# dataexplorations2026/cough_detector

Measured on AMD Instinct MI355X. Metric: 1s@16kHz clips/sec (featurise+infer), higher is better.
Workload: dtype bf16x3: split-bf16 MFMA (feature image, activations and BN-folded weights as hi+lo bf16 pairs, 3 v_mfma_f32_32x32x16_bf16 per k-step, f32 accumulate, f32 activations in HBM); featuriser f32

## Files before the change

### cough_detector_amd/csrc/featurize.hip

```cpp
#include <cmath>
#include <cstddef>
#include <cstring>
#include <type_traits>
#include <vector>

#include <hip/hip_bf16.h>

#include <cstdlib>

#include "common.h"
#include "fft256.h"
#include "internal.h"

namespace cough {
namespace {

constexpr int NS = 16000, NFFT = 512, HOP = 160, WIN = 400, NFRAMES = 101, NMEL = 64, NMFCC = 13;
constexpr int PADL = NFFT / 2;
constexpr int NBIN = 128;
constexpr int MAXW = 8;
constexpr int THREADS = 256, WAVES = THREADS / 64;
constexpr int FPW = 4;
constexpr int NGROUP = (NFRAMES + FPW - 1) / FPW;
constexpr int XROW = 17;
constexpr int XFRAME = 16 * XROW;
constexpr int NMF = NMFCC * NFRAMES;
constexpr int FIRST_PLAIN = 2, LAST_PLAIN = 98;

struct FeatTables {
    float win[NFFT];
    float2 tw256[16][16];
    float2 tw512[NBIN];
    int mel_start[NMEL];
    float mel_w[NMEL][MAXW];
    float dct_t[NMFCC + 1][NMEL];
};

constexpr size_t LDS_XCH = size_t(WAVES) * FPW * XFRAME * 4;
constexpr size_t LDS_MEL = size_t(NMEL) * NFRAMES * 4;
constexpr size_t LDS_RED = 16 * 4;
constexpr size_t LDS_TW = size_t(16) * XROW * 8;
constexpr size_t LDS_TOTAL = LDS_XCH + LDS_MEL + LDS_RED + LDS_TW;
static_assert(LDS_TOTAL * 3 <= 160 * 1024, "three workgroups per CU");
static_assert(LDS_XCH >= size_t(2) * NMF * 4, "MFCC / delta buffers alias the transpose scratch");

__device__ __forceinline__ float block_max(float v, float* red, int tid) {
    v = wave_max(v);
    __syncthreads();
    if ((tid & 63) == 0) red[tid >> 6] = v;
    __syncthreads();
    float r = red[0];
#pragma unroll
    for (int w = 1; w < WAVES; ++w) r = fmaxf(r, red[w]);
    return r;
}
__device__ __forceinline__ float block_sum(float v, float* red, int tid) {
    v = wave_sum(v);
    __syncthreads();
    if ((tid & 63) == 0) red[tid >> 6] = v;
    __syncthreads();
    float r = red[0];
#pragma unroll
    for (int w = 1; w < WAVES; ++w) r += red[w];
    return r;
}

#ifdef COUGH_K1_STAMPS
__device__ unsigned long long* g_stamp_buf = nullptr;
#define K1_STAMP(slot)                                                                      \
    do {                                                                                    \
        if (g_stamp_buf && threadIdx.x == 0)                                                \
            g_stamp_buf[(size_t)blockIdx.x * 8 + (slot)] = __builtin_amdgcn_s_memtime();    \
    } while (0)
#else
#define K1_STAMP(slot) do { } while (0)
#endif

#ifdef COUGH_K1_MARKERS
#define K1_MARK(text)                             \
    do {                                          \
        __builtin_amdgcn_sched_barrier(0);        \
        asm volatile("; K1MARK " text);           \
        __builtin_amdgcn_sched_barrier(0);        \
    } while (0)
#else
#define K1_MARK(text) do { } while (0)
#endif

using f32x16 = __attribute__((ext_vector_type(16))) float;
using bf16x8 = __attribute__((ext_vector_type(8))) __bf16;
__device__ __forceinline__ uint16_t f2bf(float f) {
    __hip_bfloat16 b = __float2bfloat16(f);
    return *reinterpret_cast<uint16_t*>(&b);
}
constexpr int ST_P1H = 22, ST_P1W = 25, ST_ROWS = 94, ST_PITCH = 106;
constexpr int ST_PER = ST_P1H * ST_P1W, ST_TILES = (ST_PER + 7) / 8;
constexpr size_t ST_IMG = size_t(ST_ROWS) * ST_PITCH * 2;
static_assert(ST_IMG <= LDS_MEL, "the bf16 feature image aliases the dB buffer");
constexpr size_t ST_X3_OFF = LDS_TOTAL - 2 * ST_IMG;
static_assert(ST_X3_OFF % 16 == 0 && ST_IMG % 4 == 0 && ST_X3_OFF >= size_t(NMF) * 4, "hi / lo images vs the MFCC buffer");

struct FullBank {
    int n_mels, n_mfcc, n_taps;
    int maxw[2];
    int n_frames, n_samples, hop;
    int cph, cph_pad, cw;
    const int *lo, *hi, *off;
    const float* w;
    const float* dct;
};
constexpr size_t full_mel_bytes(int n_mels, int n_frames = NFRAMES) { return (size_t(n_mels) * n_frames * 4 + 15) & ~size_t(15); }
constexpr int FX_ROW = FPW * 16 + 1, FX_WAVE = 16 * FX_ROW, FX_PROW = 260;
static_assert(FPW * FX_PROW <= FX_WAVE && FX_PROW >= NFFT / 2 + 2 && FX_PROW % 2 == 0, "four power rows replace the transposes");
constexpr size_t LDS_XCH_FULL = size_t(WAVES) * FX_WAVE * 4;
constexpr int FULL_MAX_MFCC = int(LDS_XCH_FULL / (size_t(2) * NFRAMES * 4));
constexpr size_t full_lds_bytes(int n_mels, int n_taps, int n_frames = NFRAMES) {
    return LDS_XCH_FULL + full_mel_bytes(n_mels, n_frames) + LDS_RED + LDS_TW + ((size_t(n_taps) * 4 + 15) & ~size_t(15));
}

#ifndef COUGH_GEO_WG_PER_CU
#define COUGH_GEO_WG_PER_CU 2
#endif
template <bool PRE_EMPH, int STEM, bool FULL = false, bool TALL = false, bool PCS = false, bool GEO = false>
__global__ __launch_bounds__(THREADS, GEO ? COUGH_GEO_WG_PER_CU : 3) void featurize_kernel(
    const float* __restrict__ wav, long long wav_stride, float* __restrict__ out, int nfeat,
    const FeatTables* __restrict__ tb, int normalize, float pre_coef, int delta_delta , int pcen, StemFuse stem, FullBank fbk,
    const float* __restrict__ full_dct ,
    float* __restrict__ peak_out ) {
    extern __shared__ __attribute__((aligned(16))) char smem[];
    static_assert(!GEO || (FULL && STEM == 0 && !TALL && !PCS), "run-time geometry: full-band instantiations without a stem");
    const int NF = GEO ? fbk.n_frames : NFRAMES, NGR = GEO ? (fbk.n_frames + FPW - 1) / FPW : NGROUP;
    const int NSMP = GEO ? fbk.n_samples : NS, HP = GEO ? fbk.hop : HOP;
    constexpr int N1A = GEO ? 0 : 1, N1B = GEO ? 16 : 15;
    const int nmel = FULL ? fbk.n_mels : NMEL, nmfcc = FULL ? fbk.n_mfcc : NMFCC, nmf = nmfcc * NF;
    const size_t lds_mel = FULL ? full_mel_bytes(nmel, NF) : LDS_MEL;
    constexpr size_t lds_xch = FULL ? LDS_XCH_FULL : LDS_XCH;
    float* xs = reinterpret_cast<float*>(smem);
    float* melbuf = reinterpret_cast<float*>(smem + lds_xch);
    float* red = reinterpret_cast<float*>(smem + lds_xch + lds_mel);
    float2* twl = reinterpret_cast<float2*>(smem + lds_xch + lds_mel + LDS_RED);
    float* c_w = reinterpret_cast<float*>(smem + lds_xch + lds_mel + LDS_RED + LDS_TW);

    const int tid = threadIdx.x, lane = tid & 63, wave = tid >> 6;
    const long long clip = blockIdx.x;
    const float* x = wav + clip * wav_stride;
    float* o = out + clip * (long long)nfeat * NF;
    const bool wr = out != nullptr;

    K1_STAMP(0);
    K1_STAMP(1);
    K1_MARK("PHASE prologue (window taps, twiddle table, mel taps to registers)");

    const int j = lane & 15, fsub = lane >> 4;
    twl[(tid >> 4) * XROW + (tid & 15)] = tb->tw256[tid >> 4][tid & 15];
    int b_lo[2] = {0, 0}, b_w[2] = {0, 0}, b_band[2] = {0, 0};
    const float* b_taps[2] = {c_w, c_w};
    int fpl1 = FPW;
    if constexpr (FULL) {
        for (int i = tid; i < fbk.n_taps; i += THREADS) c_w[i] = fbk.w[i];
        const int r = nmel - 64;
        fpl1 = r > 32 ? 4 : r > 16 ? 2 : 1;
#pragma unroll
        for (int ps = 0; ps < 2; ++ps) {
            const int mb = ps == 0 ? lane : 64 + (fpl1 == 4 ? lane : fpl1 == 2 ? (lane & 31) : (lane & 15));
            if (mb < nmel) {
                b_band[ps] = mb;
                b_lo[ps] = fbk.lo[mb];
                b_w[ps] = fbk.hi[mb] - b_lo[ps];
                b_taps[ps] = c_w + fbk.off[mb];
            } else {
                b_band[ps] = -1;
            }
        }
    }
    __syncthreads();
    const float2* tw_row = twl + j * XROW;
    const float2 tw_j = tb->tw512[j];
    float mw[MAXW];
#pragma unroll
    for (int q = 0; q < MAXW; ++q) mw[q] = tb->mel_w[lane][q];
    const int mstart = tb->mel_start[lane];

    float* myx = xs + (wave * FPW + fsub) * XFRAME;
    float* myw = xs + wave * FX_WAVE;
    float* fxw = myw + 16 * fsub + j;
    const float* fxr = myw + FX_ROW * j + 16 * fsub;
    float* prow = myw + FX_PROW * fsub;
    float run_max = -INFINITY;
    float peak = 0.f;
    float chk = 0.f;
    auto geo_plain = [&](int g) {
        return HP * (FPW * g) - PADL >= 0 && FPW * g + FPW - 1 < NF && HP * (FPW * g + FPW - 1) - PADL + NFFT <= NSMP;
    };
    [[maybe_unused]] float raw_left = 0.f;
    auto load_group = [&](int g, float2 (&raw)[16]) {
        const int t_raw = FPW * g + fsub;
        const int t = t_raw < NF ? t_raw : NF - 1;
        const int s0 = HP * t - PADL + 2 * j;
        if constexpr (GEO) {
            if (geo_plain(g)) {
#pragma unroll
                for (int n1 = 0; n1 < 16; ++n1) raw[n1] = make_float2(x[s0 + 32 * n1], x[s0 + 32 * n1 + 1]);
                if constexpr (PRE_EMPH) raw_left = s0 - 2 * j > 0 ? x[s0 - 2 * j - 1] : 0.f;
            } else {
#pragma unroll
                for (int n1 = 0; n1 < 16; ++n1) {
                    int i0 = s0 + 32 * n1, i1 = i0 + 1;
                    i0 = i0 < 0 ? -i0 : (i0 >= NSMP ? 2 * (NSMP - 1) - i0 : i0);
                    i1 = i1 < 0 ? -i1 : (i1 >= NSMP ? 2 * (NSMP - 1) - i1 : i1);
                    raw[n1] = make_float2(x[i0], x[i1]);
                }
            }
        } else
        if (FPW * g >= FIRST_PLAIN && FPW * g + FPW - 1 <= LAST_PLAIN) {
            K1_MARK("WEIGHT 0.885 (23 of 26 groups: frames inside the clip)");
#pragma unroll
            for (int n1 = 1; n1 < 15; ++n1) raw[n1] = *reinterpret_cast<const float2*>(x + s0 + 32 * n1);
            K1_MARK("ENDWEIGHT");
        } else {
            K1_MARK("WEIGHT 0.115 (3 of 26 groups: reflected edge frames)");
#pragma unroll
            for (int n1 = 1; n1 < 15; ++n1) {
                int i0 = s0 + 32 * n1, i1 = i0 + 1;
                i0 = i0 < 0 ? -i0 : (i0 >= NS ? 2 * (NS - 1) - i0 : i0);
                i1 = i1 < 0 ? -i1 : (i1 >= NS ? 2 * (NS - 1) - i1 : i1);
                raw[n1] = make_float2(x[i0], x[i1]);
            }
            K1_MARK("ENDWEIGHT");
        }
    };
    float2 raw[16];
    float peak_m = 0.f;
    auto p1_pass = [&](const float ws1, const float ws2) {
        float w_re[16], w_im[16];
        const int jw = 2 * j;
#pragma unroll
        for (int n1 = N1A; n1 < N1B; ++n1) {
            w_re[n1] = tb->win[32 * n1 + jw] * ws1 * ws2;
            w_im[n1] = tb->win[32 * n1 + jw + 1] * ws1 * ws2;
        }
        load_group(wave, raw);

        K1_MARK("LOOP 6.5 P1 four-frame groups per wave");
        for (int g = wave; g < NGR; g += WAVES) {
            K1_MARK("PHASE P1 peak + window multiply + next group's loads");
            const int t_raw = FPW * g + fsub;
            const int t = t_raw < NF ? t_raw : NF - 1;
            const int s0 = HP * t - PADL + 2 * j;
            float2 a[16];
            if constexpr (!GEO) {
// ... 237 lines not shown
                    float pw[26];
                    pcen_chunk(m2, c, q2, pw);
#pragma unroll
                    for (int k = 0; k < 26; ++k)
                        if (q0 + 26 * c + k < q2) o[m2 * NF + q0 + 26 * c + k] = pw[k];
                }
            }
        }
        const float mn = -block_max(-lmin, red, tid), mx = block_max(lmax, red, tid);
        const float rng = 1.0f / (mx - mn + 1e-8f);
#pragma unroll
        for (int c = 0; c < 2; ++c)
#pragma unroll
            for (int k = 0; k < 26; ++k)
                if (q0 + 26 * c + k < q1) o[m * NF + q0 + 26 * c + k] = (pv[c][k] - mn) * rng;
        for (int t = q0; t < q2; ++t) o[m2 * NF + t] = (o[m2 * NF + t] - mn) * rng;
        wr_mel = false;
    } else
    if (pcen) {
        const int m = tid >> 2, t0 = (tid & 3) * 26, t1 = t0 + 26 < NF ? t0 + 26 : NF;
        float p[36], pv[26];
#pragma unroll
        for (int k = 0; k < 36; ++k) {
            const int u = t0 - 5 + k;
            p[k] = (u >= 0 && u < NF) ? exp2f((melbuf[m * NF + u] - shift) * 0.33219280948873623f) : 0.f;
        }
        float lmin = INFINITY, lmax = -INFINITY;
        float s2[35];
#pragma unroll
        for (int k = 0; k < 35; ++k) s2[k] = p[k] + p[k + 1];
#pragma unroll
        for (int k = 0; k < 26; ++k) {
            const float sm = ((s2[k] + s2[k + 2]) + (s2[k + 4] + s2[k + 6])) + s2[k + 8];
            const float gain = __builtin_amdgcn_exp2f(-0.98f * __builtin_amdgcn_logf(1e-6f + sm * 0.1f));
            pv[k] = __builtin_amdgcn_sqrtf(fmaf(p[k + 5], gain, 2.0f)) - 1.41421356237309515f;
            if (t0 + k < t1) { lmin = fminf(lmin, pv[k]); lmax = fmaxf(lmax, pv[k]); }
        }
        const float mn = -block_max(-lmin, red, tid), mx = block_max(lmax, red, tid);
        const float rng = 1.0f / (mx - mn + 1e-8f);
        if (wr) {
#pragma unroll
            for (int k = 0; k < 26; ++k)
                if (t0 + k < t1) o[m * NF + t0 + k] = (pv[k] - mn) * rng;
        }
        if constexpr (PCS) {
#pragma unroll
            for (int k = 0; k < 26; ++k) pcv[k] = (pv[k] - mn) * rng;
        }
        wr_mel = false;
    }
    K1_MARK("ENDSKIP");
    K1_MARK("PHASE P2 floor + mel rows store");
    if constexpr (GEO) {
        for (int i = tid; i < nmel * NF; i += THREADS) {
            const float d = fmaxf(fmaxf(melbuf[i] - shift, -100.0f), floor_db);
            melbuf[i] = d;
            if (wr_mel) o[i] = fminf(fmaxf((d + 80.0f) * 0.0125f, 0.f), 1.f);
        }
    } else
    for (int i2 = tid; i2 < nmel * NFRAMES / 2; i2 += THREADS) {
        float2 d = reinterpret_cast<float2*>(melbuf)[i2];
        d.x = fmaxf(fmaxf(d.x - shift, -100.0f), floor_db);
        d.y = fmaxf(fmaxf(d.y - shift, -100.0f), floor_db);
        reinterpret_cast<float2*>(melbuf)[i2] = d;
        float2 v;
        v.x = fminf(fmaxf((d.x + 80.0f) * 0.0125f, 0.f), 1.f);
        v.y = fminf(fmaxf((d.y + 80.0f) * 0.0125f, 0.f), 1.f);
        if (wr_mel) reinterpret_cast<float2*>(o)[i2] = v;
    }
    __syncthreads();
    K1_STAMP(4);
    if (delta_delta == 2) return;
    K1_MARK("PHASE P2 DCT 13x64");
    float* mf = xs;
    float* dl = GEO ? melbuf : mf + nmf;
    const int tt0 = tid & 127;
    const int chalf = __builtin_amdgcn_readfirstlane(tid >> 7);
    if constexpr (FULL) {
        const int cph = fbk.cph, nch = chalf ? nmfcc - cph : cph, cbase = chalf * cph;
        auto dct_chunks = [&](auto cw_tag) {
            constexpr int CW = decltype(cw_tag)::value;
            for (int tt = tt0; tt < (GEO ? ((NF + 127) & ~127) : 128); tt += 128)
            for (int cq = 0; cq < nch; cq += CW) {
                float acc[CW];
#pragma unroll
                for (int cc = 0; cc < CW; ++cc) acc[cc] = 0.f;
                if (tt < NF) {
                    const float* drow = full_dct + (size_t(chalf) * fbk.cph_pad + cq) / CW * size_t(nmel) * 8;
#pragma unroll 8
                    for (int m = 0; m < nmel; ++m) {
                        const float v = melbuf[m * NF + tt];
#pragma unroll
                        for (int cc = 0; cc < CW; ++cc) acc[cc] = fmaf(drow[m * 8 + cc], v, acc[cc]);
                    }
#pragma unroll
                    for (int cc = 0; cc < CW; ++cc)
                        if (cq + cc < nch) mf[(cbase + cq + cc) * NF + tt] = acc[cc];
                }
            }
        };
        if (fbk.cw == 7) dct_chunks(std::integral_constant<int, 7>{});
        else if (fbk.cw == 6) dct_chunks(std::integral_constant<int, 6>{});
        else if (fbk.cw == 5) dct_chunks(std::integral_constant<int, 5>{});
        else dct_chunks(std::integral_constant<int, 4>{});
        __syncthreads();
        float ls = 0.f;
        for (int i = tid; i < nmf; i += THREADS) ls += mf[i];
        const float mean = block_sum(ls, red, tid) / float(nmf);
        float lq = 0.f;
        for (int i = tid; i < nmf; i += THREADS) {
            const float d = mf[i] - mean;
            lq += d * d;
        }
        const float sd = sqrtf(block_sum(lq, red, tid) / float(nmf - 1));
        const float rdenom = 1.0f / (sd + 1e-8f);
        K1_STAMP(5);
        for (int i = tid; i < nmf; i += THREADS) mf[i] = (mf[i] - mean) * rdenom;
    } else {
        const int c0 = chalf * 7, nc = chalf ? 6 : 7, tt = tt0;
        float acc[7] = {0.f, 0.f, 0.f, 0.f, 0.f, 0.f, 0.f};
        if (tt < NFRAMES) {
            const float* drow = &tb->dct_t[c0][0];
#pragma unroll 8
            for (int m = 0; m < NMEL; ++m) {
                const float v = melbuf[m * NFRAMES + tt];
#pragma unroll
                for (int cc = 0; cc < 7; ++cc) acc[cc] = fmaf(drow[cc * NMEL + m], v, acc[cc]);
            }
        }
        K1_MARK("PHASE P2 mean / std / z-score");
        float lsum = 0.f;
#pragma unroll
        for (int cc = 0; cc < 7; ++cc) lsum += (tt < NFRAMES && cc < nc) ? acc[cc] : 0.f;
        const float mean = block_sum(lsum, red, tid) / float(NMF);
        K1_STAMP(5);
        float lsq = 0.f;
#pragma unroll
        for (int cc = 0; cc < 7; ++cc) {
            const float d = acc[cc] - mean;
            lsq += (tt < NFRAMES && cc < nc) ? d * d : 0.f;
        }
        const float sd = sqrtf(block_sum(lsq, red, tid) / float(NMF - 1));
        const float rdenom = 1.0f / (sd + 1e-8f);
        if (tt < NFRAMES) {
#pragma unroll
            for (int cc = 0; cc < 7; ++cc)
                if (cc < nc) mf[(c0 + cc) * NFRAMES + tt] = (acc[cc] - mean) * rdenom;
        }
    }
    __syncthreads();
    K1_MARK("PHASE P2 feature image (stem) + MFCC / delta rows");
    uint16_t* img = STEM == 2 ? reinterpret_cast<uint16_t*>(smem + ST_X3_OFF) : reinterpret_cast<uint16_t*>(melbuf);
    uint16_t* img_lo = img + ST_ROWS * ST_PITCH;
    auto put = [&](int idx, float v) {
        const uint16_t hi = f2bf(v);
        img[idx] = hi;
        if constexpr (STEM == 2) img_lo[idx] = f2bf(v - __uint_as_float(uint32_t(hi) << 16));
    };
    if constexpr (TALL) {
        static_assert(!TALL || STEM == 2, "the 103-row stem: split-bf16 operands");
        constexpr int TL_P1H = 26, TL_HALF = 13, TL_PER = TL_HALF * ST_P1W, TL_ROWS = 58, TL_PLANE = TL_ROWS * ST_PITCH;
        constexpr size_t TL_IMG_OFF = (size_t(2) * NMF * 4 + 15) & ~size_t(15), TL_STASH_OFF = TL_IMG_OFF + size_t(2) * TL_PLANE * 2;
        constexpr int TL_KEEP0 = 2 * 2 * TL_HALF - 3;
        static_assert(TL_STASH_OFF % 16 == 0 && TL_STASH_OFF + size_t(NMEL - TL_KEEP0) * NFRAMES * 4 <= LDS_TOTAL, "103-row stem LDS");
        static_assert(2 * (2 * (TL_HALF - 1) + 1) + 1 + 6 < TL_ROWS && TL_P1H == 2 * TL_HALF, "partial image rows");
        constexpr int NDV = (NMEL * NFRAMES / 2 + THREADS - 1) / THREADS;
        float2 dv[NDV];
#pragma unroll
        for (int it = 0; it < NDV; ++it) {
            const int i2 = tid + it * THREADS;
            dv[it] = i2 < NMEL * NFRAMES / 2 ? reinterpret_cast<const float2*>(melbuf)[i2] : make_float2(0.f, 0.f);
        }
        float* o_mfcc = o + NMEL * NFRAMES;
        float* o_delta = o_mfcc + NMF;
        for (int item = tid; item < NMF; item += THREADS) {
            const int c = item / NFRAMES, t = item - c * NFRAMES;
            const float* row = mf + c * NFRAMES;
            const float d = (row[t < NFRAMES - 1 ? t + 1 : t] - row[t > 0 ? t - 1 : 0]) / 2.0f;
            if (wr) {
                o_mfcc[item] = row[t];
                o_delta[item] = d;
            }
            dl[item] = d;
        }
        __syncthreads();
        auto ddelta = [&](int c, int t) {
            const float* row = dl + c * NFRAMES;
            return (row[t < NFRAMES - 1 ? t + 1 : t] - row[t > 0 ? t - 1 : 0]) / 2.0f;
        };
        if (wr) {
            float* o_dd = o_delta + NMF;
            for (int item = tid; item < NMF; item += THREADS) o_dd[item] = ddelta(item / NFRAMES, item % NFRAMES);
        }
        uint16_t* timg = reinterpret_cast<uint16_t*>(smem + TL_IMG_OFF);
        float* stash = reinterpret_cast<float*>(smem + TL_STASH_OFF);
        auto tput = [&](int idx, float v) {
            const uint16_t hi = f2bf(v);
            timg[idx] = hi;
            timg[TL_PLANE + idx] = f2bf(v - __uint_as_float(uint32_t(hi) << 16));
        };
        auto zero_image = [&]() {
            for (int i = tid; i < 2 * TL_PLANE / 8; i += THREADS) reinterpret_cast<uint4*>(timg)[i] = make_uint4(0, 0, 0, 0);
            for (int i = (2 * TL_PLANE / 8) * 8 + tid; i < 2 * TL_PLANE; i += THREADS) timg[i] = 0;
            __syncthreads();
        };
        zero_image();
        if constexpr (PCS) {
            const int m = tid >> 2, t0 = (tid & 3) * 26;
#pragma unroll
            for (int k = 0; k < 26; ++k) {
                if (t0 + k < NFRAMES) {
                    if (m + 3 < TL_ROWS - 1) tput((m + 3) * ST_PITCH + t0 + k + 3, pcv[k]);
                    if (m >= TL_KEEP0) stash[(m - TL_KEEP0) * NFRAMES + t0 + k] = pcv[k];
                }
            }
        } else {
            {
#pragma unroll
                for (int it = 0; it < NDV; ++it) {
                    const int e = 2 * (tid + it * THREADS);
                    if (e < NMEL * NFRAMES) {
                        const int m0 = e / NFRAMES, t0 = e - m0 * NFRAMES;
                        const int m1 = t0 + 1 < NFRAMES ? m0 : m0 + 1, t1 = t0 + 1 < NFRAMES ? t0 + 1 : 0;
                        const float v0 = fminf(fmaxf((dv[it].x + 80.0f) * 0.0125f, 0.f), 1.f);
                        const float v1 = fminf(fmaxf((dv[it].y + 80.0f) * 0.0125f, 0.f), 1.f);
                        if (m0 + 3 < TL_ROWS - 1) tput((m0 + 3) * ST_PITCH + t0 + 3, v0);
                        if (m1 + 3 < TL_ROWS - 1) tput((m1 + 3) * ST_PITCH + t1 + 3, v1);
                        if (m0 >= TL_KEEP0) stash[(m0 - TL_KEEP0) * NFRAMES + t0] = v0;
                        if (m1 >= TL_KEEP0) stash[(m1 - TL_KEEP0) * NFRAMES + t1] = v1;
                    }
                }
            }
        }
        const int sr = lane & 31, sh = lane >> 5;
        bf16x8 bw[2][4];
#pragma unroll
        for (int pl = 0; pl < 2; ++pl)
#pragma unroll
            for (int st = 0; st < 4; ++st)
                bw[pl][st] = *reinterpret_cast<const bf16x8*>(stem.wfrag + pl * 2048 + ((st * 2 + sh) * 32 + sr) * 8);
        const float bn = stem.bias[sr];
        const int q = sr >> 2, dy = (sr >> 1) & 1, dx = sr & 1;
        float* oa = reinterpret_cast<float*>(stem.a1) + clip * (long long)(TL_P1H * ST_P1W) * 32;
#pragma unroll 1
        for (int half = 0; half < 2; ++half) {
            if (half == 1) {
                zero_image();
                for (int i = tid; i < (NMEL - TL_KEEP0) * NFRAMES; i += THREADS) {
                    const int m = i / NFRAMES, t = i - m * NFRAMES;
                    tput(m * ST_PITCH + t + 3, stash[i]);
                }
                for (int item = tid; item < NMF; item += THREADS) {
                    const int c = item / NFRAMES, t = item - c * NFRAMES;
                    tput((NMEL - TL_KEEP0 + c) * ST_PITCH + t + 3, mf[item]);
                    tput((NMEL - TL_KEEP0 + NMFCC + c) * ST_PITCH + t + 3, dl[item]);
                    tput((NMEL - TL_KEEP0 + 2 * NMFCC + c) * ST_PITCH + t + 3, ddelta(c, t));
                }
            }
            __syncthreads();
            auto tl_base = [&](int tile) -> const uint32_t* {
                int P = tile * 8 + q;
                if (P >= TL_PER) P = TL_PER - 1;
                const int ph = P / ST_P1W, pw = P - ph * ST_P1W;
                return reinterpret_cast<const uint32_t*>(timg + (2 * (2 * ph + dy) + sh) * ST_PITCH + 2 * (2 * pw + dx));
            };
            auto tl_load = [&](const uint32_t* base, bf16x8 (&fa)[2][4]) {
#pragma unroll
                for (int pl = 0; pl < 2; ++pl)
#pragma unroll
                    for (int st = 0; st < 4; ++st) {
                        const uint32_t* pp = base + pl * (TL_PLANE / 2) + st * ST_PITCH;
                        union { uint32_t u[4]; bf16x8 v; } tv;
                        tv.u[0] = pp[0]; tv.u[1] = pp[1]; tv.u[2] = pp[2]; tv.u[3] = pp[3];
                        fa[pl][st] = tv.v;
                    }
            };
            auto tl_mma = [&](const bf16x8 (&fa)[2][4], f32x16& c) {
#pragma unroll
                for (int st = 0; st < 4; ++st) {
                    c = __builtin_amdgcn_mfma_f32_32x32x16_bf16(fa[0][st], bw[0][st], c, 0, 0, 0);
                    c = __builtin_amdgcn_mfma_f32_32x32x16_bf16(fa[1][st], bw[0][st], c, 0, 0, 0);
                    c = __builtin_amdgcn_mfma_f32_32x32x16_bf16(fa[0][st], bw[1][st], c, 0, 0, 0);
                }
            };
            auto tl_store = [&](int tile, const f32x16& acc2) {
#pragma unroll
                for (int g = 0; g < 4; ++g) {
                    const int Po = tile * 8 + 2 * g + sh;
                    float v = fmaxf(fmaxf(acc2[4 * g], acc2[4 * g + 1]), fmaxf(acc2[4 * g + 2], acc2[4 * g + 3])) + bn;
                    v = fmaxf(v, 0.f);
                    if (Po < TL_PER) oa[(half * TL_PER + Po) * 32 + sr] = v;
                }
            };
            constexpr int TL_TILES = (TL_PER + 7) / 8;
            for (int ta = wave; ta < TL_TILES; ta += 2 * WAVES) {
                const int tb = ta + WAVES;
                const bool two = tb < TL_TILES;
                bf16x8 fa[2][4], fb[2][4];
                tl_load(tl_base(ta), fa);
                tl_load(tl_base(two ? tb : ta), fb);
                f32x16 ca = {0}, cb = {0};
                tl_mma(fa, ca);
                tl_mma(fb, cb);
                tl_store(ta, ca);
                if (two) tl_store(tb, cb);
            }
            __syncthreads();
        }
        return;
    }
    if constexpr (STEM != 0) {
        float2 dv[(NMEL * NFRAMES / 2 + THREADS - 1) / THREADS];
#pragma unroll
        for (int it = 0; it < (NMEL * NFRAMES / 2 + THREADS - 1) / THREADS; ++it) {
            const int i2 = tid + it * THREADS;
            dv[it] = i2 < NMEL * NFRAMES / 2 ? reinterpret_cast<const float2*>(melbuf)[i2] : make_float2(0.f, 0.f);
        }
        __syncthreads();
        constexpr int NIMG = STEM == 2 ? 2 : 1;
        for (int i = tid; i < NIMG * ST_ROWS * ST_PITCH / 8; i += THREADS) reinterpret_cast<uint4*>(img)[i] = make_uint4(0, 0, 0, 0);
        for (int i = (NIMG * ST_ROWS * ST_PITCH / 8) * 8 + tid; i < NIMG * ST_ROWS * ST_PITCH; i += THREADS) img[i] = 0;
        __syncthreads();
        if constexpr (PCS) {
            const int m = tid >> 2, t0 = (tid & 3) * 26;
#pragma unroll
            for (int k = 0; k < 26; ++k)
                if (t0 + k < NFRAMES) put((m + 3) * ST_PITCH + t0 + k + 3, pcv[k]);
        } else {
#pragma unroll
            for (int it = 0; it < (NMEL * NFRAMES / 2 + THREADS - 1) / THREADS; ++it) {
                const int e = 2 * (tid + it * THREADS);
                if (e < NMEL * NFRAMES) {
                    const int m0 = e / NFRAMES, t0 = e - m0 * NFRAMES;
                    const int m1 = t0 + 1 < NFRAMES ? m0 : m0 + 1, t1 = t0 + 1 < NFRAMES ? t0 + 1 : 0;
                    put((m0 + 3) * ST_PITCH + t0 + 3, fminf(fmaxf((dv[it].x + 80.0f) * 0.0125f, 0.f), 1.f));
                    put((m1 + 3) * ST_PITCH + t1 + 3, fminf(fmaxf((dv[it].y + 80.0f) * 0.0125f, 0.f), 1.f));
                }
            }
        }
    }
    float* o_mfcc = o + nmel * NF;
    float* o_delta = o_mfcc + nmf;
    for (int item = tid; item < nmf; item += THREADS) {
        const int c = item / NF, t = item - c * NF;
        const float* row = mf + c * NF;
        const float d = (row[t < NF - 1 ? t + 1 : t] - row[t > 0 ? t - 1 : 0]) / 2.0f;
        if (wr) {
            o_mfcc[item] = row[t];
            o_delta[item] = d;
        }
        if (delta_delta == 1) dl[item] = d;
        if constexpr (STEM != 0) {
            put((NMEL + c + 3) * ST_PITCH + t + 3, row[t]);
            put((NMEL + NMFCC + c + 3) * ST_PITCH + t + 3, d);
        }
    }
    K1_STAMP(6);
    if (delta_delta == 1 && wr) {
        __syncthreads();
        float* o_dd = o_delta + nmf;
        for (int item = tid; item < nmf; item += THREADS) {
            const int c = item / NF, t = item - c * NF;
            const float* row = dl + c * NF;
            o_dd[item] = (row[t < NF - 1 ? t + 1 : t] - row[t > 0 ? t - 1 : 0]) / 2.0f;
        }
    }
    if constexpr (STEM != 0) {
        __syncthreads();
        K1_MARK("PHASE K2 stem MFMA + pool + store");
        constexpr int NP = STEM == 2 ? 2 : 1;
        const int sr = lane & 31, sh = lane >> 5;
        bf16x8 bw[NP][4];
#pragma unroll
        for (int pl = 0; pl < NP; ++pl)
#pragma unroll
            for (int st = 0; st < 4; ++st)
                bw[pl][st] = *reinterpret_cast<const bf16x8*>(stem.wfrag + pl * 2048 + ((st * 2 + sh) * 32 + sr) * 8);
        const float bn = stem.bias[sr];
        const int q = sr >> 2, dy = (sr >> 1) & 1, dx = sr & 1;
        using out_t = std::conditional_t<STEM == 2, float, uint16_t>;
        out_t* oa = reinterpret_cast<out_t*>(stem.a1) + clip * (long long)ST_PER * 32;
        auto frag_base = [&](int tile) -> const uint32_t* {
            int P = tile * 8 + q;
            if (P >= ST_PER) P = ST_PER - 1;
            const int ph = P / ST_P1W, pw = P - ph * ST_P1W;
            return reinterpret_cast<const uint32_t*>(img + (2 * (2 * ph + dy) + sh) * ST_PITCH + 2 * (2 * pw + dx));
        };
        auto load_frags = [&](const uint32_t* base, bf16x8 (&a)[NP][4]) {
#pragma unroll
            for (int pl = 0; pl < NP; ++pl)
#pragma unroll
                for (int st = 0; st < 4; ++st) {
                    const uint32_t* p = base + pl * (ST_ROWS * ST_PITCH / 2) + st * ST_PITCH;
                    union { uint32_t u[4]; bf16x8 v; } t;
                    t.u[0] = p[0]; t.u[1] = p[1]; t.u[2] = p[2]; t.u[3] = p[3];
                    a[pl][st] = t.v;
                }
        };
        auto mma = [&](const bf16x8 (&a)[NP][4], f32x16& c) {
#pragma unroll
            for (int st = 0; st < 4; ++st) {
                c = __builtin_amdgcn_mfma_f32_32x32x16_bf16(a[0][st], bw[0][st], c, 0, 0, 0);
                if constexpr (STEM == 2) {
                    c = __builtin_amdgcn_mfma_f32_32x32x16_bf16(a[1][st], bw[0][st], c, 0, 0, 0);
                    c = __builtin_amdgcn_mfma_f32_32x32x16_bf16(a[0][st], bw[1][st], c, 0, 0, 0);
                }
            }
        };
        auto epilogue = [&](int tile, const f32x16& acc2, bool guard) {
#pragma unroll
            for (int g = 0; g < 4; ++g) {
                const int Po = tile * 8 + 2 * g + sh;
                float v = fmaxf(fmaxf(acc2[4 * g], acc2[4 * g + 1]), fmaxf(acc2[4 * g + 2], acc2[4 * g + 3])) + bn;
                v = fmaxf(v, 0.f);
                if (!guard || Po < ST_PER) {
                    if constexpr (STEM == 2) oa[Po * 32 + sr] = v;
                    else oa[Po * 32 + sr] = f2bf(v);
                }
            }
        };
        static_assert(ST_TILES == 17 * WAVES + 1, "stem tile split");
        for (int it = 0; it < 16; it += 2) {
            const int ta = wave + WAVES * it, tbb = ta + WAVES;
            bf16x8 fa[NP][4], fb[NP][4];
            load_frags(frag_base(ta), fa);
            load_frags(frag_base(tbb), fb);
            f32x16 ca = {0}, cb = {0};
            mma(fa, ca);
            mma(fb, cb);
            epilogue(ta, ca, false);
            epilogue(tbb, cb, false);
        }
        {
            const int ta = wave + WAVES * 16;
            const bool last = wave == 0;
            bf16x8 fa[NP][4], fb[NP][4];
            load_frags(frag_base(ta), fa);
            load_frags(frag_base(last ? ST_TILES - 1 : ta), fb);
            f32x16 ca = {0}, cb = {0};
            mma(fa, ca);
            mma(fb, cb);
            epilogue(ta, ca, false);
            if (last) epilogue(ST_TILES - 1, cb, true);
        }
        K1_STAMP(7);
    }
}

}
}

struct cough_featurizer {
    cough_feat_config cfg;
    cough::FeatTables* d_tables;
    float* d_win_full;
    int nfeat;
    int nbase;
    cough::ContrastCfg contrast;
    int n_cus;
    int path;
    char* d_full;
    cough::FullBank full;
    cough::GenFeat* gen;
};

namespace cough {
namespace {
bool geo_basic(const cough_feat_config& c) {
    return c.n_fft == NFFT && c.win_length >= 1 && c.win_length <= NFFT && c.hop_length >= 1 && c.n_mels >= 2 && c.n_mels <= 128 &&
           (!c.use_mfcc || (c.n_mfcc >= 1 && c.n_mfcc <= c.n_mels));
}
bool geo_fits(const cough_feat_config& c, int n_taps, int n) {
    if (n <= NFFT / 2) return false;
    const long long T = n / c.hop_length + 1;
    const bool covered = c.hop_length <= NFFT / 2 || (c.hop_length <= NFFT && (T - 1) * c.hop_length + NFFT / 2 >= n);
    return covered && T <= 1024 && (!c.use_pcen || T <= 208) && (!c.use_mfcc || size_t(c.n_mfcc) * T * 4 <= LDS_XCH_FULL) &&
           full_lds_bytes(c.n_mels, n_taps, int(T)) <= 80 * 1024;
}

using K1Fn = decltype(&featurize_kernel<false, 0>);
struct K1Entry {
    bool pe;
    int stem;
    bool full, tall, pcs, geo;
    K1Fn fn;
};
#define K1(PE, STEM, FULL, TALL, PCS, GEO) {PE, STEM, FULL, TALL, PCS, GEO, featurize_kernel<PE, STEM, FULL, TALL, PCS, GEO>}
#define K1_X3(FULL, PCS) K1(false, 2, FULL, false, PCS, false), K1(false, 2, FULL, true, PCS, false), \
                        K1(true, 2, FULL, false, PCS, false), K1(true, 2, FULL, true, PCS, false)
const K1Entry K1_TABLE[] = {
    K1(false, 0, true, false, false, false), K1(true, 0, true, false, false, false),
    K1_X3(true, false), K1_X3(true, true),
    K1(false, 0, true, false, false, true), K1(true, 0, true, false, false, true),
    K1_X3(false, false), K1_X3(false, true),
    K1(false, 1, false, false, false, false),
    K1(true, 0, false, false, false, false), K1(false, 0, false, false, false, false),
};
#undef K1_X3
#undef K1
static_assert(sizeof(K1_TABLE) / sizeof(K1_TABLE[0]) == 23, "one entry per instantiation");
K1Fn k1_kernel(bool pe, int stem, bool full, bool tall, bool pcs, bool geo) {
    for (const K1Entry& k : K1_TABLE)
        if (k.pe == pe && k.stem == stem && k.full == full && k.tall == tall && k.pcs == pcs && k.geo == geo) return k.fn;
    return nullptr;
}

bool shipped_stft(const cough_feat_config& c) {
    return c.n_fft == NFFT && c.hop_length == HOP && c.win_length == WIN && c.segment_samples == NS;
}
struct Band {
    int first, last;
};
std::vector<Band> scan_bands(const cough_feat_config& c, const float* mel_fb) {
    std::vector<Band> bands(c.n_fft == NFFT && c.n_mels > 0 ? c.n_mels : 0, Band{-1, -1});
    for (int k = 0; !bands.empty() && k <= NFFT / 2; ++k)
        for (int m = 0; m < c.n_mels; ++m)
            if (mel_fb[k * c.n_mels + m] != 0.f) {
                if (bands[m].first < 0) bands[m].first = k;
                bands[m].last = k;
            }
    return bands;
}

int segment_path(const cough_feat_config& c, const std::vector<Band>& bands, int n_taps) {
    bool stft = shipped_stft(c);
    for (int i = 0; c.use_spectral_contrast && i < c.n_contrast_bands; ++i)
        stft = stft && c.contrast_edges[i + 1] - c.contrast_edges[i] <= 128;
    bool regs = stft && c.n_mels == NMEL && c.n_mfcc == NMFCC;
    for (const Band& b : bands) regs = regs && (b.first < 0 || (b.last < NBIN && b.last - b.first < MAXW));
    if (regs) return COUGH_PATH_TUNED;
    const bool basic = geo_basic(c);
    if (stft && basic && c.n_mels % 2 == 0 && (!c.use_mfcc || c.n_mfcc <= FULL_MAX_MFCC) && (!c.use_pcen || c.n_mels == NMEL) &&
        full_lds_bytes(c.n_mels, n_taps, NFRAMES) <= 80 * 1024)
        return COUGH_PATH_TUNED_FULLBAND;
    return basic && geo_fits(c, n_taps, c.segment_samples) ? COUGH_PATH_TUNED_GEOMETRY : COUGH_PATH_GENERIC;
}

FeatTables shipped_tables(const cough_feat_config& c, const float* window, const float* mel_fb, const float* dct,
                          const std::vector<Band>& bands, int path) {
    FeatTables t{};
    const double PI = 3.14159265358979323846;
    if (shipped_stft(c) || geo_basic(c)) {
        const int left = (NFFT - c.win_length) / 2;
        for (int n = 0; n < c.win_length; ++n) t.win[left + n] = window[n];
        for (int jj = 0; jj < 16; ++jj)
            for (int k1 = 0; k1 < 16; ++k1) {
                const double a = -2.0 * PI * double(jj * k1) / 256.0;
                t.tw256[jj][k1] = make_float2(float(std::cos(a)), float(std::sin(a)));
            }
        for (int k = 0; k < NBIN; ++k) {
            const double a = -2.0 * PI * double(k) / 512.0;
            t.tw512[k] = make_float2(float(std::cos(a)), float(std::sin(a)));
        }
    }
    if (path == COUGH_PATH_TUNED) {
        for (int m = 0; m < NMEL; ++m) {
            int first = bands[m].first < 0 ? 0 : bands[m].first;
            if (first > NBIN - MAXW) first = NBIN - MAXW;
            t.mel_start[m] = first;
            for (int q = 0; q < MAXW; ++q) t.mel_w[m][q] = 0.25f * mel_fb[(first + q) * NMEL + m];
        }
        for (int c2 = 0; c2 < NMFCC; ++c2)
            for (int m = 0; m < NMEL; ++m) t.dct_t[c2][m] = dct[m * NMFCC + c2];
    }
    return t;
}

struct HostBank {
    FullBank fb{};
    std::vector<int> lo, hi, off;
    std::vector<float> taps, dct;
};
HostBank csr_bank(const cough_feat_config& c, const float* mel_fb, const float* dct, const std::vector<Band>& bands) {
    HostBank h;
    FullBank& fb = h.fb;
    const int nm = c.n_mels, nc = c.use_mfcc ? c.n_mfcc : 1;
    fb.n_mels = nm;
    fb.n_mfcc = nc;
    for (int m = 0; m < nm; ++m) {
        const int first = bands[m].first < 0 ? 0 : bands[m].first, last = bands[m].first < 0 ? -1 : bands[m].last;
        const int lo2 = first & ~1, hi2 = last >= first ? (last + 2) & ~1 : lo2;
        h.lo.push_back(lo2);
        h.hi.push_back(hi2);
        h.off.push_back(hi2 > lo2 ? int(h.taps.size()) : 0);
        for (int k = lo2; k < hi2; ++k) h.taps.push_back(k >= first && k <= last ? 0.25f * mel_fb[k * nm + m] : 0.f);
        const int w = (hi2 - lo2 + 3) / 4 * 4;
        if (w > fb.maxw[m >> 6]) fb.maxw[m >> 6] = w;
    }
    if (h.taps.size() < 2) h.taps.assign(2, 0.f);
    fb.n_taps = int(h.taps.size());
    fb.cph = (nc + 1) / 2;
    const int n_chunks = (fb.cph + 6) / 7;
    fb.cw = (fb.cph + n_chunks - 1) / n_chunks;
// ... 219 lines not shown
```

Baseline: 6.560 million.

## Build stem image in column-pair dwords and hand-schedule stem LDS fragment reads

The feature image is now written as packed bf16 pairs per dword, straight from the mel buffer into registers. Only the border is zeroed instead of the whole image, and the MFCC/delta rows are written in the same paired layout. The stem MFMA loop computes LDS addresses with a multiply-shift divide-by-25 and inline ds_read_b32 with immediate offsets. Partial lgkmcnt waits let the first tile's MFMAs start while the second tile's loads are still in flight, and the pool/bias/ReLU epilogue is folded into one max chain. The aim is to cut LDS store traffic, barriers and address arithmetic in the featuriser tail. The cost is brittle inline asm and hand-counted waitcnts.

```diff
diff --git a/cough_detector_amd/csrc/featurize.hip b/cough_detector_amd/csrc/featurize.hip
--- a/cough_detector_amd/csrc/featurize.hip
+++ b/cough_detector_amd/csrc/featurize.hip
@@ -93,9 +93,42 @@
     __hip_bfloat16 b = __float2bfloat16(f);
     return *reinterpret_cast<uint16_t*>(&b);
 }
+__device__ __forceinline__ float stem_pool_bias_relu(float a, float b, float c, float d, float bias, float neg_bias) {
+    return fmaxf(fmaxf(fmaxf(fmaxf(a, b), c), d), neg_bias) + bias;
+}
+__device__ __forceinline__ uint32_t bf16_pair(float a, float b) {
+    using f32x2 = __attribute__((ext_vector_type(2))) float;
+    using bf16x2 = __attribute__((ext_vector_type(2))) __bf16;
+    const bf16x2 h = __builtin_convertvector(f32x2{a, b}, bf16x2);
+    return __builtin_bit_cast(uint32_t, h);
+}
+__device__ __forceinline__ uint32_t lds_addr(const void* p) {
+    return uint32_t(reinterpret_cast<uintptr_t>((const __attribute__((address_space(3))) void*)p));
+}
+__device__ __forceinline__ uint32_t lds_read_b32(uint32_t base, int off) {
+    uint32_t r;
+    asm volatile("ds_read_b32 %0, %1 offset:%2" : "=v"(r) : "v"(base), "n"(off));
+    return r;
+}
+template <int N, int NP>
+__device__ __forceinline__ void frags_wait(bf16x8 (&a)[NP][4]) {
+    static_assert(N == 0 || N == 15, "lgkmcnt");
+#pragma unroll
+    for (int pl = 0; pl < NP; ++pl) {
+        if constexpr (N == 0) asm volatile("s_waitcnt lgkmcnt(0)" : "+v"(a[pl][0]), "+v"(a[pl][1]), "+v"(a[pl][2]), "+v"(a[pl][3]));
+        else asm volatile("s_waitcnt lgkmcnt(15)" : "+v"(a[pl][0]), "+v"(a[pl][1]), "+v"(a[pl][2]), "+v"(a[pl][3]));
+    }
+}
 constexpr int ST_P1H = 22, ST_P1W = 25, ST_ROWS = 94, ST_PITCH = 106;
 constexpr int ST_PER = ST_P1H * ST_P1W, ST_TILES = (ST_PER + 7) / 8;
 constexpr size_t ST_IMG = size_t(ST_ROWS) * ST_PITCH * 2;
+__device__ __host__ constexpr uint32_t stem_div25(uint32_t P) { return (P * 41u) >> 10; }
+constexpr bool stem_div25_ok() {
+    for (uint32_t P = 0; P < uint32_t(ST_TILES * 8); ++P)
+        if (stem_div25(P) != P / ST_P1W) return false;
+    return true;
+}
+static_assert(ST_P1W == 25 && stem_div25_ok(), "stem_div25");
 static_assert(ST_IMG <= LDS_MEL, "the bf16 feature image aliases the dB buffer");
 constexpr size_t ST_X3_OFF = LDS_TOTAL - 2 * ST_IMG;
 static_assert(ST_X3_OFF % 16 == 0 && ST_IMG % 4 == 0 && ST_X3_OFF >= size_t(NMF) * 4, "hi / lo images vs the MFCC buffer");
@@ -639,7 +672,7 @@
     K1_MARK("PHASE P2 feature image (stem) + MFCC / delta rows");
     uint16_t* img = STEM == 2 ? reinterpret_cast<uint16_t*>(smem + ST_X3_OFF) : reinterpret_cast<uint16_t*>(melbuf);
     uint16_t* img_lo = img + ST_ROWS * ST_PITCH;
-    auto put = [&](int idx, float v) {
+    [[maybe_unused]] auto put = [&](int idx, float v) {
         const uint16_t hi = f2bf(v);
         img[idx] = hi;
         if constexpr (STEM == 2) img_lo[idx] = f2bf(v - __uint_as_float(uint32_t(hi) << 16));
@@ -796,39 +829,71 @@
         }
         return;
     }
+    constexpr int IMG_PAIRS = (NFRAMES + 2) / 2, IMG_RG = THREADS / IMG_PAIRS, IMG_DW = ST_PITCH / 2;
+    static_assert(NFRAMES % 2 == 1 && 2 * IMG_PAIRS + 2 + 2 == ST_PITCH && IMG_RG >= 1, "column pairs of the stem image");
+    const int ij = tid % IMG_PAIRS, ir = tid / IMG_PAIRS;
+    uint32_t* imgd = reinterpret_cast<uint32_t*>(img);
+    [[maybe_unused]] auto put2 = [&](int dword, float a, float b) {
+        const uint32_t hi = bf16_pair(a, b);
+        imgd[dword] = hi;
+        if constexpr (STEM == 2)
+            imgd[int(ST_IMG / 4) + dword] = bf16_pair(a - __uint_as_float(hi << 16), b - __uint_as_float(hi & 0xffff0000u));
+    };
     if constexpr (STEM != 0) {
-        float2 dv[(NMEL * NFRAMES / 2 + THREADS - 1) / THREADS];
-#pragma unroll
-        for (int it = 0; it < (NMEL * NFRAMES / 2 + THREADS - 1) / THREADS; ++it) {
-            const int i2 = tid + it * THREADS;
-            dv[it] = i2 < NMEL * NFRAMES / 2 ? reinterpret_cast<const float2*>(melbuf)[i2] : make_float2(0.f, 0.f);
-        }
-        __syncthreads();
         constexpr int NIMG = STEM == 2 ? 2 : 1;
-        for (int i = tid; i < NIMG * ST_ROWS * ST_PITCH / 8; i += THREADS) reinterpret_cast<uint4*>(img)[i] = make_uint4(0, 0, 0, 0);
-        for (int i = (NIMG * ST_ROWS * ST_PITCH / 8) * 8 + tid; i < NIMG * ST_ROWS * ST_PITCH; i += THREADS) img[i] = 0;
-        __syncthreads();
         if constexpr (PCS) {
+            __syncthreads();
+            for (int i = tid; i < NIMG * ST_ROWS * ST_PITCH / 8; i += THREADS) reinterpret_cast<uint4*>(img)[i] = make_uint4(0, 0, 0, 0);
+            for (int i = (NIMG * ST_ROWS * ST_PITCH / 8) * 8 + tid; i < NIMG * ST_ROWS * ST_PITCH; i += THREADS) img[i] = 0;
+            __syncthreads();
             const int m = tid >> 2, t0 = (tid & 3) * 26;
 #pragma unroll
             for (int k = 0; k < 26; ++k)
                 if (t0 + k < NFRAMES) put((m + 3) * ST_PITCH + t0 + k + 3, pcv[k]);
         } else {
-#pragma unroll
-            for (int it = 0; it < (NMEL * NFRAMES / 2 + THREADS - 1) / THREADS; ++it) {
-                const int e = 2 * (tid + it * THREADS);
-                if (e < NMEL * NFRAMES) {
-                    const int m0 = e / NFRAMES, t0 = e - m0 * NFRAMES;
-                    const int m1 = t0 + 1 < NFRAMES ? m0 : m0 + 1, t1 = t0 + 1 < NFRAMES ? t0 + 1 : 0;
-                    put((m0 + 3) * ST_PITCH + t0 + 3, fminf(fmaxf((dv[it].x + 80.0f) * 0.0125f, 0.f), 1.f));
-                    put((m1 + 3) * ST_PITCH + t1 + 3, fminf(fmaxf((dv[it].y + 80.0f) * 0.0125f, 0.f), 1.f));
+            constexpr int NK = (NMEL + IMG_RG - 1) / IMG_RG;
+            float v0[NK], v1[NK];
+            static_assert(IMG_RG * (NK - 1) < NMEL && IMG_RG + IMG_RG * (NK - 2) < NMEL, "only the last round is short");
+            const float* src1 = melbuf + ir * NFRAMES + 2 * ij;
+            const float* src0 = src1 - (ij > 0 ? 1 : 0);
+#pragma unroll
+            for (int k = 0; k < NK; ++k) {
+                const int off = (k == NK - 1 ? min(ir + IMG_RG * k, NMEL - 1) - ir : IMG_RG * k) * NFRAMES;
+                v0[k] = ij > 0 ? fminf(fmaxf((src0[off] + 80.0f) * 0.0125f, 0.f), 1.f) : 0.f;
+                v1[k] = fminf(fmaxf((src1[off] + 80.0f) * 0.0125f, 0.f), 1.f);
+            }
+            __syncthreads();
+            constexpr int TOP = 3 * IMG_DW, EDGE = TOP + (ST_ROWS - 3 - (NMEL + 2 * NMFCC)) * IMG_DW;
+            static_assert(EDGE <= THREADS && NMEL + 2 * NMFCC <= THREADS, "one border dword per thread");
+#pragma unroll
+            for (int pl = 0; pl < NIMG; ++pl) {
+                uint32_t* z = imgd + pl * int(ST_IMG / 4);
+                if (tid < EDGE) z[tid < TOP ? tid : (NMEL + 2 * NMFCC) * IMG_DW + tid] = 0;
+                if (tid < NMEL + 2 * NMFCC) z[(tid + 3) * IMG_DW] = z[(tid + 3) * IMG_DW + IMG_DW - 1] = 0;
+            }
+            const int dst = (ir + 3) * IMG_DW + ij + 1;
+#pragma unroll
+            for (int k = 0; k < NK; ++k)
+                if (ir < IMG_RG && ir + IMG_RG * k < NMEL) put2(dst + k * IMG_RG * IMG_DW, v0[k], v1[k]);
+        }
+        {
+            const int i0 = max(2 * ij - 2, 0), i1 = max(2 * ij - 1, 0), i2 = 2 * ij, i3 = min(2 * ij + 1, NFRAMES - 1);
+#pragma unroll
+            for (int k = 0; k < (NMFCC + IMG_RG - 1) / IMG_RG; ++k) {
+                const int c = ir + IMG_RG * k;
+                const float* row = mf + min(c, NMFCC - 1) * NFRAMES;
+                const float x0 = row[i0], x1 = row[i1], x2 = row[i2], x3 = row[i3];
+                if (ir < IMG_RG && c < NMFCC) {
+                    const int dw = (NMEL + c + 3) * IMG_DW + ij + 1;
+                    put2(dw, ij > 0 ? x1 : 0.f, x2);
+                    put2(dw + NMFCC * IMG_DW, ij > 0 ? (x2 - x0) / 2.0f : 0.f, (x3 - x1) / 2.0f);
                 }
             }
         }
     }
     float* o_mfcc = o + nmel * NF;
     float* o_delta = o_mfcc + nmf;
-    for (int item = tid; item < nmf; item += THREADS) {
+    for (int item = tid; item < (STEM == 0 || wr || delta_delta == 1 ? nmf : 0); item += THREADS) {
         const int c = item / NF, t = item - c * NF;
         const float* row = mf + c * NF;
         const float d = (row[t < NF - 1 ? t + 1 : t] - row[t > 0 ? t - 1 : 0]) / 2.0f;
@@ -837,10 +902,6 @@
             o_delta[item] = d;
         }
         if (delta_delta == 1) dl[item] = d;
-        if constexpr (STEM != 0) {
-            put((NMEL + c + 3) * ST_PITCH + t + 3, row[t]);
-            put((NMEL + NMFCC + c + 3) * ST_PITCH + t + 3, d);
-        }
     }
     K1_STAMP(6);
     if (delta_delta == 1 && wr) {
@@ -863,24 +924,23 @@
 #pragma unroll
             for (int st = 0; st < 4; ++st)
                 bw[pl][st] = *reinterpret_cast<const bf16x8*>(stem.wfrag + pl * 2048 + ((st * 2 + sh) * 32 + sr) * 8);
-        const float bn = stem.bias[sr];
+        const float bn = stem.bias[sr], nbn = -bn;
         const int q = sr >> 2, dy = (sr >> 1) & 1, dx = sr & 1;
         using out_t = std::conditional_t<STEM == 2, float, uint16_t>;
         out_t* oa = reinterpret_cast<out_t*>(stem.a1) + clip * (long long)ST_PER * 32;
-        auto frag_base = [&](int tile) -> const uint32_t* {
-            int P = tile * 8 + q;
-            if (P >= ST_PER) P = ST_PER - 1;
-            const int ph = P / ST_P1W, pw = P - ph * ST_P1W;
-            return reinterpret_cast<const uint32_t*>(img + (2 * (2 * ph + dy) + sh) * ST_PITCH + 2 * (2 * pw + dx));
+        const uint32_t lane_base = lds_addr(img) + uint32_t(((2 * dy + sh) * ST_PITCH + 2 * dx) * 2);
+        auto frag_base = [&](int P) -> uint32_t {
+            return lane_base + 8u * uint32_t(P) + uint32_t(4 * ST_PITCH * 2 - 8 * ST_P1W) * stem_div25(uint32_t(P));
         };
-        auto load_frags = [&](const uint32_t* base, bf16x8 (&a)[NP][4]) {
-#pragma unroll
-            for (int pl = 0; pl < NP; ++pl)
-#pragma unroll
-                for (int st = 0; st < 4; ++st) {
-                    const uint32_t* p = base + pl * (ST_ROWS * ST_PITCH / 2) + st * ST_PITCH;
+        auto load_frags = [&](uint32_t base, bf16x8 (&a)[NP][4]) {
+#pragma unroll
+            for (int st = 0; st < 4; ++st)
+#pragma unroll
+                for (int pl = 0; pl < NP; ++pl) {
                     union { uint32_t u[4]; bf16x8 v; } t;
-                    t.u[0] = p[0]; t.u[1] = p[1]; t.u[2] = p[2]; t.u[3] = p[3];
+#pragma unroll
+                    for (int k = 0; k < 4; ++k)
+                        t.u[k] = lds_read_b32(base, pl * int(ST_IMG) + st * (2 * ST_PITCH * 2) + 4 * k);
                     a[pl][st] = t.v;
                 }
         };
@@ -898,8 +958,7 @@
 #pragma unroll
             for (int g = 0; g < 4; ++g) {
                 const int Po = tile * 8 + 2 * g + sh;
-                float v = fmaxf(fmaxf(acc2[4 * g], acc2[4 * g + 1]), fmaxf(acc2[4 * g + 2], acc2[4 * g + 3])) + bn;
-                v = fmaxf(v, 0.f);
+                const float v = stem_pool_bias_relu(acc2[4 * g], acc2[4 * g + 1], acc2[4 * g + 2], acc2[4 * g + 3], bn, nbn);
                 if (!guard || Po < ST_PER) {
                     if constexpr (STEM == 2) oa[Po * 32 + sr] = v;
                     else oa[Po * 32 + sr] = f2bf(v);
@@ -907,13 +966,16 @@
             }
         };
         static_assert(ST_TILES == 17 * WAVES + 1, "stem tile split");
-        for (int it = 0; it < 16; it += 2) {
+        int P = wave * 8 + q;
+        for (int it = 0; it < 16; it += 2, P += 16 * WAVES) {
             const int ta = wave + WAVES * it, tbb = ta + WAVES;
             bf16x8 fa[NP][4], fb[NP][4];
-            load_frags(frag_base(ta), fa);
-            load_frags(frag_base(tbb), fb);
+            load_frags(frag_base(P), fa);
+            load_frags(frag_base(P + 8 * WAVES), fb);
             f32x16 ca = {0}, cb = {0};
+            frags_wait<15, NP>(fa);
             mma(fa, ca);
+            frags_wait<0, NP>(fb);
             mma(fb, cb);
             epilogue(ta, ca, false);
             epilogue(tbb, cb, false);
@@ -922,10 +984,12 @@
             const int ta = wave + WAVES * 16;
             const bool last = wave == 0;
             bf16x8 fa[NP][4], fb[NP][4];
-            load_frags(frag_base(ta), fa);
-            load_frags(frag_base(last ? ST_TILES - 1 : ta), fb);
+            load_frags(frag_base(P), fa);
+            load_frags(frag_base(last ? min((ST_TILES - 1) * 8 + q, ST_PER - 1) : P), fb);
             f32x16 ca = {0}, cb = {0};
+            frags_wait<15, NP>(fa);
             mma(fa, ca);
+            frags_wait<0, NP>(fb);
             mma(fb, cb);
             epilogue(ta, ca, false);
             if (last) epilogue(ST_TILES - 1, cb, true);
```

Result: no change. 6.597 million, median of 6 (+0.6%).
